# igormq/aes-lac-2018

Measured on AMD Instinct MI355X. Metric: train frames/sec, DeepSpeech2 5xBiGRU-800, higher is better.
Workload: dtype f32

## Files before the change

### aes-lac-2018_amd/csrc/gemm.hip

```cpp
#include <stdlib.h>

#include <type_traits>

#include "ds2_common.h"
#include "split_bf16.h"

namespace {

constexpr int BM = 128, BN = 128, BK = 16;
constexpr int NI = BK / 8;
constexpr int LDT = 132;

constexpr int OOB = 0x7FFFFFF0;
typedef unsigned int u32x4 __attribute__((ext_vector_type(4)));

__device__ __forceinline__ f32x4 bload4(__amdgpu_buffer_rsrc_t rs, int byte_off) {
    return __builtin_bit_cast(f32x4, __builtin_amdgcn_raw_buffer_load_b128(rs, byte_off, 0, 0));
}
__device__ __forceinline__ float bload1(__amdgpu_buffer_rsrc_t rs, int byte_off) {
    return __builtin_bit_cast(float, __builtin_amdgcn_raw_buffer_load_b32(rs, byte_off, 0, 0));
}

template <bool KCONTIG, bool VEC>
__device__ __forceinline__ void load_slab(__amdgpu_buffer_rsrc_t rs, int ld, int x0, int xmax, int k0, int kmax,
                                          int tid, f32x4 (&r)[NI]) {
    if (KCONTIG) {
        const int kq = (tid & (BK / 4 - 1)) * 4;
#pragma unroll
        for (int i = 0; i < NI; ++i) {
            const int x = x0 + tid / (BK / 4) + (1024 / BK) * i;
            const int k = k0 + kq;
            const int off = (x * ld + k) * 4;
            if (VEC) {
                r[i] = bload4(rs, (x < xmax && k + 3 < kmax) ? off : OOB);
            } else {
#pragma unroll
                for (int c = 0; c < 4; ++c) r[i][c] = bload1(rs, (x < xmax && k + c < kmax) ? off + 4 * c : OOB);
            }
        }
    } else {
        const int xq = (tid & 31) * 4;
#pragma unroll
        for (int i = 0; i < NI; ++i) {
            const int k = k0 + (tid >> 5) + 8 * i;
            const int x = x0 + xq;
            const int off = (k * ld + x) * 4;
            if (VEC) {
                if (x + 3 < xmax || x >= xmax) {
                    r[i] = bload4(rs, (k < kmax && x < xmax) ? off : OOB);
                } else {
#pragma unroll
                    for (int c = 0; c < 4; ++c) r[i][c] = bload1(rs, (k < kmax && x + c < xmax) ? off + 4 * c : OOB);
                }
            } else {
#pragma unroll
                for (int c = 0; c < 4; ++c) r[i][c] = bload1(rs, (k < kmax && x + c < xmax) ? off + 4 * c : OOB);
            }
        }
    }
}

template <bool KCONTIG>
__device__ __forceinline__ void slab_voffsets(int ld, int x0, int xmax, int tid, int (&voff)[NI]) {
#pragma unroll
    for (int i = 0; i < NI; ++i) {
        if (KCONTIG) {
            const int x = x0 + tid / (BK / 4) + (1024 / BK) * i;
            voff[i] = x < xmax ? (x * ld + (tid & (BK / 4 - 1)) * 4) * 4 : OOB;
        } else {
            const int x = x0 + (tid & 31) * 4;
            voff[i] = x < xmax ? (((tid >> 5) + 8 * i) * ld + x) * 4 : OOB;
        }
    }
}
template <bool KCONTIG>
__device__ __forceinline__ int slab_soffset(int ld, int k0) {
    return KCONTIG ? k0 * 4 : k0 * ld * 4;
}
__device__ __forceinline__ void load_slab_fast(__amdgpu_buffer_rsrc_t rs, const int (&voff)[NI], int soff, f32x4 (&r)[NI]) {
#pragma unroll
    for (int i = 0; i < NI; ++i)
        r[i] = __builtin_bit_cast(f32x4, __builtin_amdgcn_raw_buffer_load_b128(rs, voff[i], soff, 0));
}

template <bool KCONTIG>
__device__ __forceinline__ void store_slab(float* __restrict__ lds, int tid, const f32x4 (&r)[NI]) {
    if (KCONTIG) {
        const int kq = (tid & (BK / 4 - 1)) * 4;
#pragma unroll
        for (int i = 0; i < NI; ++i) {
            const int x = tid / (BK / 4) + (1024 / BK) * i;
#pragma unroll
            for (int c = 0; c < 4; ++c) lds[(kq + c) * LDT + x] = r[i][c];
        }
    } else {
        const int xq = (tid & 31) * 4;
#pragma unroll
        for (int i = 0; i < NI; ++i) {
            const int k = (tid >> 5) + 8 * i;
            *reinterpret_cast<f32x4*>(&lds[k * LDT + xq]) = r[i];
        }
    }
}

__device__ __forceinline__ int xcd_tile(int wg, int nwg) {
    const int xcd = wg & 7, idx = wg >> 3;
    const int qd = nwg >> 3, rm = nwg & 7;
    return (xcd < rm ? xcd * (qd + 1) : rm * (qd + 1) + (xcd - rm) * qd) + idx;
}

template <bool A_KCONTIG, bool B_KCONTIG, bool VEC, int MODE>
__device__ __forceinline__ void gemm_tile_body(float (&lds)[2][2][BK * LDT], int M, int N, const float* __restrict__ A, int lda,
                                               const float* __restrict__ B, int ldb, float* __restrict__ C, int ldc,
                                               float beta, int use_atomic, unsigned int a_bytes, unsigned int b_bytes, int m0,
                                               int n0, int kbeg, int kend) {
    const int tid = threadIdx.x;
    const int lane = tid & 63;
    const int wave = tid >> 6;
    const int wm = wave >> 1, wn = wave & 1;
    constexpr int NI_ = MODE == 0 ? 2 : 1, NJ_ = MODE == 0 ? 2 : MODE;
    const int arow = MODE == 0 ? wm * 64 : wave * 32, bcol = MODE == 0 ? wn * 64 : 0;

    f32x16 acc[NI_][NJ_];
#pragma unroll
    for (int i = 0; i < NI_; ++i)
#pragma unroll
        for (int j = 0; j < NJ_; ++j)
#pragma unroll
            for (int r = 0; r < 16; ++r) acc[i][j][r] = 0.f;

    const __amdgpu_buffer_rsrc_t rsa = __builtin_amdgcn_make_buffer_rsrc(const_cast<float*>(A), 0, a_bytes, 0x00020000);
    const __amdgpu_buffer_rsrc_t rsb = __builtin_amdgcn_make_buffer_rsrc(const_cast<float*>(B), 0, b_bytes, 0x00020000);
    f32x4 ra[NI], rb[NI];
    const int nslab = (kend - kbeg + BK - 1) / BK;
    if (nslab > 0) {
        load_slab<A_KCONTIG, VEC>(rsa, lda, m0, M, kbeg, kend, tid, ra);
        load_slab<B_KCONTIG, VEC>(rsb, ldb, n0, N, kbeg, kend, tid, rb);
        store_slab<A_KCONTIG>(lds[0][0], tid, ra);
        store_slab<B_KCONTIG>(lds[0][1], tid, rb);
    }
    __syncthreads();

    const int lr = lane & 31, lh = lane >> 5;
    for (int s = 0; s < nslab; ++s) {
        const int cur = s & 1;
#ifndef DS2_GEMM_ABL
#define DS2_GEMM_ABL 0
#endif
        if (s + 1 < nslab && !(DS2_GEMM_ABL & 2)) {
            load_slab<A_KCONTIG, VEC>(rsa, lda, m0, M, kbeg + (s + 1) * BK, kend, tid, ra);
            load_slab<B_KCONTIG, VEC>(rsb, ldb, n0, N, kbeg + (s + 1) * BK, kend, tid, rb);
        }
        const float* as = lds[cur][0] + arow + lr;
        const float* bs = lds[cur][1] + bcol + lr;
#pragma unroll
        for (int kk = 0; kk < BK; kk += 2) {
            float a[NI_], b[NJ_];
#pragma unroll
            for (int i = 0; i < NI_; ++i) a[i] = (DS2_GEMM_ABL & 4) ? ra[0][0] + kk : as[(kk + lh) * LDT + 32 * i];
#pragma unroll
            for (int j = 0; j < NJ_; ++j) b[j] = (DS2_GEMM_ABL & 4) ? rb[0][0] + kk : bs[(kk + lh) * LDT + 32 * j];
#pragma unroll
            for (int i = 0; i < NI_; ++i)
#pragma unroll
                for (int j = 0; j < NJ_; ++j) acc[i][j] = __builtin_amdgcn_mfma_f32_32x32x2f32(a[i], b[j], acc[i][j], 0, 0, 0);
        }
        if (s + 1 < nslab && !(DS2_GEMM_ABL & 1)) {
            store_slab<A_KCONTIG>(lds[cur ^ 1][0], tid, ra);
            store_slab<B_KCONTIG>(lds[cur ^ 1][1], tid, rb);
        }
        __syncthreads();
    }

#pragma unroll
    for (int i = 0; i < NI_; ++i)
#pragma unroll
        for (int j = 0; j < NJ_; ++j) {
            const int n = n0 + bcol + j * 32 + lr;
            if (n >= N) continue;
#pragma unroll
            for (int r = 0; r < 16; ++r) {
                const int m = m0 + arow + i * 32 + (r & 3) + 8 * (r >> 2) + 4 * lh;
                if (m < M) {
                    float* c = C + (size_t)m * ldc + n;
                    if (use_atomic)
                        atomicAdd(c, acc[i][j][r]);
                    else
                        *c = (beta != 0.f) ? acc[i][j][r] + beta * (*c) : acc[i][j][r];
                }
            }
        }
}

template <bool A_KCONTIG, bool B_KCONTIG, bool VEC>
__device__ __forceinline__ void gemm_tile(int M, int N, int K, const float* __restrict__ A, int lda,
                                          const float* __restrict__ B, int ldb, float* __restrict__ C, int ldc, float beta,
                                          int tiles_n, int k_per_split, int use_atomic, unsigned int a_bytes,
                                          unsigned int b_bytes, int tile, int split) {
    __shared__ __attribute__((aligned(16))) float lds[2][2][BK * LDT];
    const int m0 = (tile / tiles_n) * BM;
    const int n0 = (tile % tiles_n) * BN;
    const int kbeg = split * k_per_split;
    const int kend = min(K, kbeg + k_per_split);
    const int ncols = N - n0;
    if (ncols <= 32)
        gemm_tile_body<A_KCONTIG, B_KCONTIG, VEC, 1>(lds, M, N, A, lda, B, ldb, C, ldc, beta, use_atomic, a_bytes, b_bytes, m0,
                                                     n0, kbeg, kend);
    else if (ncols <= 64)
        gemm_tile_body<A_KCONTIG, B_KCONTIG, VEC, 2>(lds, M, N, A, lda, B, ldb, C, ldc, beta, use_atomic, a_bytes, b_bytes, m0,
                                                     n0, kbeg, kend);
    else
        gemm_tile_body<A_KCONTIG, B_KCONTIG, VEC, 0>(lds, M, N, A, lda, B, ldb, C, ldc, beta, use_atomic, a_bytes, b_bytes, m0,
                                                     n0, kbeg, kend);
}

template <bool A_KCONTIG, bool B_KCONTIG, bool VEC>
__global__ __launch_bounds__(256, 2) void gemm_f32_kernel(int M, int N, int K, const float* __restrict__ A,
                                                          int lda, const float* __restrict__ B, int ldb,
                                                          float* __restrict__ C, int ldc, float beta,
                                                          int tiles_n, int k_per_split, int use_atomic,
                                                          unsigned int a_bytes, unsigned int b_bytes) {
    gemm_tile<A_KCONTIG, B_KCONTIG, VEC>(M, N, K, A, lda, B, ldb, C, ldc, beta, tiles_n, k_per_split, use_atomic, a_bytes,
                                         b_bytes, xcd_tile(blockIdx.x, gridDim.x), blockIdx.y);
}

struct GemmGroup {
    const float* A[4];
    const float* B[4];
    float* C[4];
    int M[4], lda[4], ldb[4], ldc[4];
    unsigned int a_bytes[4], b_bytes[4];
};
template <bool VEC>
__global__ __launch_bounds__(256, 2) void gemm_f32_tn_group_kernel(GemmGroup g, int N, int K, int tiles_n, int k_per_split) {
    const int p = blockIdx.z;
    const int tiles = ((g.M[p] + BM - 1) / BM) * tiles_n;
    if ((int)blockIdx.x >= tiles) return;
    gemm_tile<false, false, VEC>(g.M[p], N, K, g.A[p], g.lda[p], g.B[p], g.ldb[p], g.C[p], g.ldc[p], 0.f, tiles_n, k_per_split,
                                 1, g.a_bytes[p], g.b_bytes[p], blockIdx.x, blockIdx.y);
}

template <bool A_KCONTIG, bool B_KCONTIG, bool VEC>
__global__ __launch_bounds__(256, 2) void gemm_f32_v2_kernel(int M, int N, int K, const float* __restrict__ A, int lda,
                                                             const float* __restrict__ B, int ldb,
                                                             float* __restrict__ C, int ldc, float beta, int tiles_n,
                                                             int dp_tiles, int sk_units, int sk_total,
                                                             unsigned int a_bytes, unsigned int b_bytes) {
    __shared__ __attribute__((aligned(16))) float lds[3][2][BK * LDT];
    const int tid = threadIdx.x, lane = tid & 63, wave = tid >> 6;
    const int wm = wave >> 1, wn = wave & 1;
    const int lr = lane & 31, lh = lane >> 5;
    const int nslab_all = (K + BK - 1) / BK;
    const __amdgpu_buffer_rsrc_t rsa = __builtin_amdgcn_make_buffer_rsrc(const_cast<float*>(A), 0, a_bytes, 0x00020000);
    const __amdgpu_buffer_rsrc_t rsb = __builtin_amdgcn_make_buffer_rsrc(const_cast<float*>(B), 0, b_bytes, 0x00020000);

    int u0 = 0, u1 = 0;
    const bool is_dp = (int)blockIdx.x < dp_tiles;
    if (!is_dp) {
        u0 = ((int)blockIdx.x - dp_tiles) * sk_units;
        u1 = min(u0 + sk_units, sk_total);
    }
#pragma unroll 1
    for (int piece = 0; piece < 2; ++piece) {
        int tile, s_beg, s_end;
        if (is_dp) {
            if (piece == 1) break;
            const int nwg = dp_tiles, xcd = blockIdx.x & 7, idx = blockIdx.x >> 3;
            const int qd = nwg >> 3, rm = nwg & 7;
            tile = (xcd < rm ? xcd * (qd + 1) : rm * (qd + 1) + (xcd - rm) * qd) + idx;
            s_beg = 0;
            s_end = nslab_all;
        } else {
            if (u0 >= u1) break;
            tile = dp_tiles + u0 / nslab_all;
            s_beg = u0 % nslab_all;
            s_end = min(nslab_all, s_beg + (u1 - u0));
            u0 += s_end - s_beg;
        }
        const int m0 = (tile / tiles_n) * BM, n0 = (tile % tiles_n) * BN;
        const int nslab = s_end - s_beg;
        const int kbeg = s_beg * BK, kend = min(K, s_end * BK);

        f32x16 acc[2][2];
#pragma unroll
        for (int i = 0; i < 2; ++i)
#pragma unroll
            for (int j = 0; j < 2; ++j)
#pragma unroll
                for (int r = 0; r < 16; ++r) acc[i][j][r] = 0.f;

        f32x4 ra[NI], rb[NI];
        int va[NI], vb[NI];
        slab_voffsets<A_KCONTIG>(lda, m0, M, tid, va);
        slab_voffsets<B_KCONTIG>(ldb, n0, N, tid, vb);
        const bool fast_ok = VEC && (A_KCONTIG || (M & 3) == 0) && (B_KCONTIG || (N & 3) == 0);
        auto fetch = [&](int k0) {
            if (fast_ok && k0 + BK <= kend) {
                load_slab_fast(rsa, va, slab_soffset<A_KCONTIG>(lda, k0), ra);
                load_slab_fast(rsb, vb, slab_soffset<B_KCONTIG>(ldb, k0), rb);
            } else {
                load_slab<A_KCONTIG, VEC>(rsa, lda, m0, M, k0, kend, tid, ra);
                load_slab<B_KCONTIG, VEC>(rsb, ldb, n0, N, k0, kend, tid, rb);
            }
        };
        __syncthreads();
        fetch(kbeg);
        store_slab<A_KCONTIG>(lds[0][0], tid, ra);
        store_slab<B_KCONTIG>(lds[0][1], tid, rb);
        if (nslab > 1) {
            fetch(kbeg + BK);
            store_slab<A_KCONTIG>(lds[1][0], tid, ra);
            store_slab<B_KCONTIG>(lds[1][1], tid, rb);
        }
        if (nslab > 2) {
            fetch(kbeg + 2 * BK);
        }
        __syncthreads();
        const int aoff = wm * 64 + lr + lh * LDT, boff = wn * 64 + lr + lh * LDT;
        float pa0 = lds[0][0][aoff], pa1 = lds[0][0][aoff + 32], pb0 = lds[0][1][boff], pb1 = lds[0][1][boff + 32];
        int cur = 0;
        for (int s = 0; s < nslab; ++s) {
            const float* as = lds[cur][0] + aoff;
            const float* bs = lds[cur][1] + boff;
            const int nxt = cur == 2 ? 0 : cur + 1, nx2 = nxt == 2 ? 0 : nxt + 1;
#pragma unroll
            for (int kk = 0; kk < BK; kk += 2) {
                const float a0 = pa0, a1 = pa1, b0 = pb0, b1 = pb1;
                if (kk + 2 < BK) {
                    pa0 = as[(kk + 2) * LDT];
                    pa1 = as[(kk + 2) * LDT + 32];
                    pb0 = bs[(kk + 2) * LDT];
                    pb1 = bs[(kk + 2) * LDT + 32];
                }
                acc[0][0] = __builtin_amdgcn_mfma_f32_32x32x2f32(a0, b0, acc[0][0], 0, 0, 0);
                acc[0][1] = __builtin_amdgcn_mfma_f32_32x32x2f32(a0, b1, acc[0][1], 0, 0, 0);
                acc[1][0] = __builtin_amdgcn_mfma_f32_32x32x2f32(a1, b0, acc[1][0], 0, 0, 0);
                acc[1][1] = __builtin_amdgcn_mfma_f32_32x32x2f32(a1, b1, acc[1][1], 0, 0, 0);
                __builtin_amdgcn_sched_group_barrier(0x100, 2, 0);
                __builtin_amdgcn_sched_group_barrier(0x008, 4, 0);
                if (kk == BK - 6 && s + 2 < nslab) {
                    store_slab<A_KCONTIG>(lds[nx2][0], tid, ra);
                    store_slab<B_KCONTIG>(lds[nx2][1], tid, rb);
                    if (s + 3 < nslab) fetch(kbeg + (s + 3) * BK);
                }
            }
            if (s + 1 < nslab) {
                pa0 = lds[nxt][0][aoff];
                pa1 = lds[nxt][0][aoff + 32];
                pb0 = lds[nxt][1][boff];
                pb1 = lds[nxt][1][boff + 32];
            }
            __syncthreads();
            cur = nxt;
        }

        const bool atomic = !is_dp;
#pragma unroll
        for (int i = 0; i < 2; ++i)
#pragma unroll
            for (int j = 0; j < 2; ++j) {
                const int n = n0 + wn * 64 + j * 32 + lr;
                if (n >= N) continue;
#pragma unroll
                for (int r = 0; r < 16; ++r) {
                    const int m = m0 + wm * 64 + i * 32 + (r & 3) + 8 * (r >> 2) + 4 * lh;
                    if (m < M) {
                        float* c = C + (size_t)m * ldc + n;
                        if (atomic)
                            atomicAdd(c, acc[i][j][r]);
                        else
                            *c = (beta != 0.f) ? acc[i][j][r] + beta * (*c) : acc[i][j][r];
                    }
                }
            }
    }
}

constexpr int SP = SPLIT_PITCH;
constexpr int SPLIT_TILE_BYTES = 128 * SP;

template <bool KCONTIG>
__device__ __forceinline__ void split_voffsets(int ld, int x0, int xmax, int tid, int (&voff)[2]) {
    if (KCONTIG) {
#pragma unroll
        for (int i = 0; i < 2; ++i) {
            const int x = x0 + (tid >> 2) + 64 * i;
            voff[i] = x < xmax ? (x * ld + (tid & 3) * 4) * 4 : OOB;
        }
    } else {
        const int x = x0 + (tid & 127);
        voff[0] = voff[1] = x < xmax ? (8 * (tid >> 7) * ld + x) * 4 : OOB;
    }
}
template <bool KCONTIG>
__device__ __forceinline__ void split_load(__amdgpu_buffer_rsrc_t rs, const int (&voff)[2], int ld, int k0, float (&r)[8]) {
    if (KCONTIG) {
#pragma unroll
        for (int i = 0; i < 2; ++i) {
            const f32x4 v = __builtin_bit_cast(f32x4, __builtin_amdgcn_raw_buffer_load_b128(rs, voff[i], k0 * 4, 0));
#pragma unroll
            for (int c = 0; c < 4; ++c) r[4 * i + c] = v[c];
        }
    } else {
#pragma unroll
        for (int c = 0; c < 8; ++c)
            r[c] = __builtin_bit_cast(float, __builtin_amdgcn_raw_buffer_load_b32(rs, voff[0], (k0 + c) * ld * 4, 0));
    }
}
template <bool KCONTIG>
__device__ __forceinline__ void split_store(char* __restrict__ lds, int tid, const float (&r)[8]) {
    if (KCONTIG) {
#pragma unroll
        for (int i = 0; i < 2; ++i) {
            unsigned int p[3][2];
            split3(r[4 * i], r[4 * i + 1], p[0][0], p[1][0], p[2][0]);
            split3(r[4 * i + 2], r[4 * i + 3], p[0][1], p[1][1], p[2][1]);
            char* row = lds + ((tid >> 2) + 64 * i) * SP + (tid & 3) * 8;
#pragma unroll
            for (int q = 0; q < 3; ++q) *reinterpret_cast<uint2*>(row + 32 * q) = make_uint2(p[q][0], p[q][1]);
        }
    } else {
        unsigned int p[3][4];
#pragma unroll
        for (int c = 0; c < 4; ++c) split3(r[2 * c], r[2 * c + 1], p[0][c], p[1][c], p[2][c]);
        char* row = lds + (tid & 127) * SP + (tid >> 7) * 16;
#pragma unroll
        for (int q = 0; q < 3; ++q) *reinterpret_cast<uint4*>(row + 32 * q) = make_uint4(p[q][0], p[q][1], p[q][2], p[q][3]);
    }
}

template <bool A_KCONTIG, bool B_KCONTIG, int MODE, int NPROD>
__device__ __forceinline__ void gemm_split_tile_body(char (&lds)[2][2][SPLIT_TILE_BYTES], int M, int N,
                                                     const float* __restrict__ A, int lda, const float* __restrict__ B,
                                                     int ldb, float* __restrict__ C, int ldc, float beta, int use_atomic,
                                                     unsigned int a_bytes, unsigned int b_bytes, int m0, int n0, int kbeg,
                                                     int kend) {
    const int tid = threadIdx.x;
    const int lane = tid & 63;
    const int wave = tid >> 6;
    const int wm = wave >> 1, wn = wave & 1;
    constexpr int NI_ = MODE == 0 ? 2 : 1, NJ_ = MODE == 0 ? 2 : MODE;
    const int arow = MODE == 0 ? wm * 64 : wave * 32, bcol = MODE == 0 ? wn * 64 : 0;

    f32x16 acc[NI_][NJ_], acc_lo[NI_][NJ_];
#pragma unroll
    for (int i = 0; i < NI_; ++i)
#pragma unroll
        for (int j = 0; j < NJ_; ++j)
#pragma unroll
            for (int r = 0; r < 16; ++r) acc[i][j][r] = acc_lo[i][j][r] = 0.f;

    const __amdgpu_buffer_rsrc_t rsa = __builtin_amdgcn_make_buffer_rsrc(const_cast<float*>(A), 0, a_bytes, 0x00020000);
    const __amdgpu_buffer_rsrc_t rsb = __builtin_amdgcn_make_buffer_rsrc(const_cast<float*>(B), 0, b_bytes, 0x00020000);
    float ra[2][8], rb[2][8];
    int va[2], vb[2];
    split_voffsets<A_KCONTIG>(lda, m0, M, tid, va);
    split_voffsets<B_KCONTIG>(ldb, n0, N, tid, vb);
    const int nslab = (kend - kbeg + BK - 1) / BK;
    if (nslab > 0) {
        split_load<A_KCONTIG>(rsa, va, lda, kbeg, ra[0]);
        split_load<B_KCONTIG>(rsb, vb, ldb, kbeg, rb[0]);
    }
    if (nslab > 1) {
        split_load<A_KCONTIG>(rsa, va, lda, kbeg + BK, ra[1]);
        split_load<B_KCONTIG>(rsb, vb, ldb, kbeg + BK, rb[1]);
    }
    if (nslab > 0) {
        split_store<A_KCONTIG>(lds[0][0], tid, ra[0]);
        split_store<B_KCONTIG>(lds[0][1], tid, rb[0]);
    }
    __syncthreads();

    const int lr = lane & 31, lh = lane >> 5;
    const int a_off = (arow + lr) * SP + lh * 16, b_off = (bcol + lr) * SP + lh * 16;
    auto slab = [&](int s, auto PAR) {
        constexpr int cur = decltype(PAR)::value;
        if (!(DS2_GEMM_ABL & 2)) {
        split_load<A_KCONTIG>(rsa, va, lda, kbeg + (s + 2) * BK, ra[cur]);
        split_load<B_KCONTIG>(rsb, vb, ldb, kbeg + (s + 2) * BK, rb[cur]);
        }
        const char* as = lds[cur][0] + a_off;
        const char* bs = lds[cur][1] + b_off;
        bf16x8 a[NI_][3], b[NJ_][3];
#pragma unroll
        for (int i = 0; i < NI_; ++i)
#pragma unroll
            for (int q = 0; q < 3; ++q)
                a[i][q] = (DS2_GEMM_ABL & 4) ? __builtin_bit_cast(bf16x8, f32x4{ra[0][0] + q, ra[0][1], ra[0][2], ra[0][3] + i})
                                             : *reinterpret_cast<const bf16x8*>(as + i * 32 * SP + q * 32);
#pragma unroll
        for (int j = 0; j < NJ_; ++j)
#pragma unroll
            for (int q = 0; q < 3; ++q)
                b[j][q] = (DS2_GEMM_ABL & 4) ? __builtin_bit_cast(bf16x8, f32x4{rb[0][0] + q, rb[0][1], rb[0][2], rb[0][3] + j})
                                             : *reinterpret_cast<const bf16x8*>(bs + j * 32 * SP + q * 32);
#pragma unroll
        for (int i = 0; i < NI_; ++i)
#pragma unroll
            for (int j = 0; j < NJ_; ++j) {
                split_mfma2<NPROD>(a[i], b[j], acc[i][j], acc_lo[i][j]);
            }
        if (!(DS2_GEMM_ABL & 1)) {
        split_store<A_KCONTIG>(lds[cur ^ 1][0], tid, ra[cur ^ 1]);
        split_store<B_KCONTIG>(lds[cur ^ 1][1], tid, rb[cur ^ 1]);
        }
        constexpr int NMFMA = NI_ * NJ_ * NPROD, VPM = (96 + NMFMA - 1) / NMFMA, WEVERY = NMFMA >= 8 ? NMFMA / 8 : 1;
        __builtin_amdgcn_sched_group_barrier(0x020, (A_KCONTIG ? 2 : 8) + (B_KCONTIG ? 2 : 8), 0);
        __builtin_amdgcn_sched_group_barrier(0x100, 3 * (NI_ + NJ_), 0);
#pragma unroll
        for (int g = 0; g < NMFMA; ++g) {
            __builtin_amdgcn_sched_group_barrier(0x008, 1, 0);
            __builtin_amdgcn_sched_group_barrier(0x002, VPM, 0);
            if (g % WEVERY == WEVERY - 1) __builtin_amdgcn_sched_group_barrier(0x200, NMFMA >= 8 ? 1 : 8 / NMFMA + 1, 0);
        }
        __syncthreads();
    };
    for (int s = 0; s < nslab; s += 2) {
        slab(s, std::integral_constant<int, 0>{});
        if (s + 1 < nslab) slab(s + 1, std::integral_constant<int, 1>{});
    }
#pragma unroll
    for (int i = 0; i < NI_; ++i)
#pragma unroll
        for (int j = 0; j < NJ_; ++j)
#pragma unroll
            for (int r = 0; r < 16; ++r) acc[i][j][r] += acc_lo[i][j][r];

#pragma unroll
    for (int i = 0; i < NI_; ++i)
#pragma unroll
        for (int j = 0; j < NJ_; ++j) {
            const int n = n0 + bcol + j * 32 + lr;
            if (n >= N) continue;
#pragma unroll
            for (int r = 0; r < 16; ++r) {
                const int m = m0 + arow + i * 32 + (r & 3) + 8 * (r >> 2) + 4 * lh;
                if (m < M) {
                    float* c = C + (size_t)m * ldc + n;
                    if (use_atomic)
                        atomicAdd(c, acc[i][j][r]);
                    else
                        *c = (beta != 0.f) ? acc[i][j][r] + beta * (*c) : acc[i][j][r];
                }
            }
        }
}

template <bool A_KCONTIG, bool B_KCONTIG, int NPROD>
__device__ __forceinline__ void gemm_split_tile(int M, int N, int K, const float* __restrict__ A, int lda,
                                                const float* __restrict__ B, int ldb, float* __restrict__ C, int ldc,
                                                float beta, int tiles_n, int k_per_split, int use_atomic,
                                                unsigned int a_bytes, unsigned int b_bytes, int tile, int split) {
    __shared__ __attribute__((aligned(16))) char lds[2][2][SPLIT_TILE_BYTES];
    const int m0 = (tile / tiles_n) * BM;
    const int n0 = (tile % tiles_n) * BN;
    const int kbeg = split * k_per_split;
    const int kend = min(K, kbeg + k_per_split);
    const int ncols = N - n0;
    if (ncols <= 32)
        gemm_split_tile_body<A_KCONTIG, B_KCONTIG, 1, NPROD>(lds, M, N, A, lda, B, ldb, C, ldc, beta, use_atomic, a_bytes,
                                                             b_bytes, m0, n0, kbeg, kend);
    else if (ncols <= 64)
        gemm_split_tile_body<A_KCONTIG, B_KCONTIG, 2, NPROD>(lds, M, N, A, lda, B, ldb, C, ldc, beta, use_atomic, a_bytes,
                                                             b_bytes, m0, n0, kbeg, kend);
    else
        gemm_split_tile_body<A_KCONTIG, B_KCONTIG, 0, NPROD>(lds, M, N, A, lda, B, ldb, C, ldc, beta, use_atomic, a_bytes,
                                                             b_bytes, m0, n0, kbeg, kend);
}

template <bool A_KCONTIG, bool B_KCONTIG, int NPROD>
__global__ __launch_bounds__(256, 2) void gemm_bf16x_kernel(int M, int N, int K, const float* __restrict__ A, int lda,
                                                            const float* __restrict__ B, int ldb, float* __restrict__ C,
                                                            int ldc, float beta, int tiles_n, int k_per_split,
                                                            int use_atomic, unsigned int a_bytes, unsigned int b_bytes) {
    gemm_split_tile<A_KCONTIG, B_KCONTIG, NPROD>(M, N, K, A, lda, B, ldb, C, ldc, beta, tiles_n, k_per_split, use_atomic,
                                                 a_bytes, b_bytes, xcd_tile(blockIdx.x, gridDim.x), blockIdx.y);
}
template <int NPROD>
__global__ __launch_bounds__(256, 2) void gemm_bf16x_tn_group_kernel(GemmGroup g, int N, int K, int tiles_n, int k_per_split) {
    const int p = blockIdx.z;
    const int tiles = ((g.M[p] + BM - 1) / BM) * tiles_n;
    if ((int)blockIdx.x >= tiles) return;
    gemm_split_tile<false, false, NPROD>(g.M[p], N, K, g.A[p], g.lda[p], g.B[p], g.ldb[p], g.C[p], g.ldc[p], 0.f, tiles_n,
                                         k_per_split, 1, g.a_bytes[p], g.b_bytes[p], blockIdx.x, blockIdx.y);
}

inline int& gemm_split_mode_ref() {
    static int mode = [] {
        const char* e = getenv("DS2_GEMM_SPLIT");
        const int v = e ? atoi(e) : 6;
        return (v == 6 || v == 9) ? v : 0;
    }();
    return mode;
}
inline int gemm_split_mode() { return gemm_split_mode_ref(); }

inline void zero_rows(float* C, int ldc, int N, int rows, hipStream_t st) {
    if (rows <= 0) return;
    if (ldc == N)
        (void)hipMemsetAsync(C, 0, (size_t)rows * N * sizeof(float), st);
    else
        (void)hipMemset2DAsync(C, (size_t)ldc * sizeof(float), 0, (size_t)N * sizeof(float), rows, st);
}

inline int gemm_slots() {
    static int slots[64] = {0};
    int dev = 0;
    if (hipGetDevice(&dev) != hipSuccess || dev < 0 || dev >= 64) return 512;
    if (slots[dev] == 0) {
        int n = 0;
        if (hipDeviceGetAttribute(&n, hipDeviceAttributeMultiprocessorCount, dev) != hipSuccess || n <= 0) n = 256;
        slots[dev] = 2 * n;
    }
    return slots[dev];
}

template <bool AK, bool BKc>
int launch(int M, int N, int K, const float* A, int lda, const float* B, int ldb, float* C, int ldc, float beta,
           int split_k, hipStream_t st) {
    const int tm = ds2_cdiv(M, BM), tn = ds2_cdiv(N, BN);
    if (split_k == 0) {
        const int tiles = tm * tn;
        split_k = 1;
        if ((tiles < 512 && K >= 512) || (tiles < 2048 && K >= 2048)) {
            static const int env_target = ds2_tune_env("DS2_GEMM_SPLIT_TARGET") ? atoi(ds2_tune_env("DS2_GEMM_SPLIT_TARGET")) : 0;
            const int target = env_target > 0 ? env_target : (gemm_split_mode() != 0 ? 1024 : 8192);
            split_k = target / tiles;
            const int max_split = K / 320 > 1 ? K / 320 : 1;
            if (split_k > max_split) split_k = max_split;
            if (split_k > 32) split_k = 32;
        }
    }
    if (split_k < 1) split_k = 1;
    if (gemm_split_mode() != 0 && (lda % 4 == 0) && (ldb % 4 == 0) && (((uintptr_t)A & 15) == 0) && (((uintptr_t)B & 15) == 0) &&
        ((!AK && !BKc) || K % BK == 0)) {
        int kper = ds2_cdiv(ds2_cdiv(K, split_k), BK) * BK;
        if (kper < BK) kper = BK;
        const int nsplit = ds2_cdiv(K, kper);
        const unsigned long long abytes = 4ull * (AK ? (unsigned long long)(M - 1) * lda + K : (unsigned long long)(K - 1) * lda + M);
        const unsigned long long bbytes = 4ull * (BKc ? (unsigned long long)(N - 1) * ldb + K : (unsigned long long)(K - 1) * ldb + N);
        if (abytes >= 0x7FFFFFF0ull || bbytes >= 0x7FFFFFF0ull) return -1;
        dim3 grid(tm * tn, nsplit), block(256);
        const int atomic = nsplit > 1 ? 1 : 0;
        if (atomic && beta == 0.f) zero_rows(C, ldc, N, M, st);
        if (gemm_split_mode() == 6)
            hipLaunchKernelGGL((gemm_bf16x_kernel<AK, BKc, 6>), grid, block, 0, st, M, N, K, A, lda, B, ldb, C, ldc, beta, tn,
                               kper, atomic, (unsigned int)abytes, (unsigned int)bbytes);
        else
            hipLaunchKernelGGL((gemm_bf16x_kernel<AK, BKc, 9>), grid, block, 0, st, M, N, K, A, lda, B, ldb, C, ldc, beta, tn,
                               kper, atomic, (unsigned int)abytes, (unsigned int)bbytes);
        return 0;
    }
    const bool vec0 = (lda % 4 == 0) && (ldb % 4 == 0) && (((uintptr_t)A & 15) == 0) && (((uintptr_t)B & 15) == 0) &&
                      ((!AK && !BKc) || K % 4 == 0);
    static const bool v2_on = !(ds2_tune_env("DS2_GEMM_V2") && ds2_tune_env("DS2_GEMM_V2")[0] == '0');
    const int tiles_all = tm * tn, slots_all = gemm_slots();
    if (split_k == 1 && v2_on && tiles_all > slots_all && tiles_all % slots_all != 0 && ds2_cdiv(K, BK) >= 16 && beta == 0.f) {
        const unsigned long long abytes = 4ull * (AK ? (unsigned long long)(M - 1) * lda + K : (unsigned long long)(K - 1) * lda + M);
        const unsigned long long bbytes = 4ull * (BKc ? (unsigned long long)(N - 1) * ldb + K : (unsigned long long)(K - 1) * ldb + N);
        if (abytes >= 0x7FFFFFF0ull || bbytes >= 0x7FFFFFF0ull) return -1;
        const int tiles = tm * tn, slots = gemm_slots(), nslab = ds2_cdiv(K, BK);
        int dp = tiles, sk_wgs = 0, sk_units = 0, sk_total = 0;
        const int rem = tiles % slots;
        const bool hybrid = tiles > slots && rem != 0 && nslab >= 16 && beta == 0.f;
        if (hybrid) {
            dp = tiles - rem;
            sk_total = rem * nslab;
            sk_wgs = sk_total / 16 < slots ? sk_total / 16 : slots;
            if (sk_wgs < 1) sk_wgs = 1;
            sk_units = ds2_cdiv(sk_total, sk_wgs);
            if (sk_units > nslab) {
                sk_units = nslab;
            }
            sk_wgs = ds2_cdiv(sk_total, sk_units);
            const int r0 = (dp / tn) * BM;
            zero_rows(C + (size_t)r0 * ldc, ldc, N, M - r0, st);
        }
        dim3 grid(dp + sk_wgs), block(256);
        if (vec0)
            hipLaunchKernelGGL((gemm_f32_v2_kernel<AK, BKc, true>), grid, block, 0, st, M, N, K, A, lda, B, ldb, C, ldc,
                               beta, tn, dp, sk_units, sk_total, (unsigned int)abytes, (unsigned int)bbytes);
        else
            hipLaunchKernelGGL((gemm_f32_v2_kernel<AK, BKc, false>), grid, block, 0, st, M, N, K, A, lda, B, ldb, C, ldc,
                               beta, tn, dp, sk_units, sk_total, (unsigned int)abytes, (unsigned int)bbytes);
        return 0;
    }
    int kper = ds2_cdiv(ds2_cdiv(K, split_k), BK) * BK;
    if (kper < BK) kper = BK;
    const int nsplit = ds2_cdiv(K, kper);
    const bool vec = (lda % 4 == 0) && (ldb % 4 == 0) && (((uintptr_t)A & 15) == 0) && (((uintptr_t)B & 15) == 0) &&
                     ((!AK && !BKc) || K % 4 == 0);
    const unsigned long long abytes = 4ull * (AK ? (unsigned long long)(M - 1) * lda + K : (unsigned long long)(K - 1) * lda + M);
    const unsigned long long bbytes = 4ull * (BKc ? (unsigned long long)(N - 1) * ldb + K : (unsigned long long)(K - 1) * ldb + N);
    if (abytes >= 0x7FFFFFF0ull || bbytes >= 0x7FFFFFF0ull) return -1;
    dim3 grid(tm * tn, nsplit), block(256);
    const int atomic = nsplit > 1 ? 1 : 0;
    if (atomic && beta == 0.f)
        zero_rows(C, ldc, N, M, st);
    if (vec)
        hipLaunchKernelGGL((gemm_f32_kernel<AK, BKc, true>), grid, block, 0, st, M, N, K, A, lda, B, ldb, C, ldc,
                           beta, tn, kper, atomic, (unsigned int)abytes, (unsigned int)bbytes);
    else
        hipLaunchKernelGGL((gemm_f32_kernel<AK, BKc, false>), grid, block, 0, st, M, N, K, A, lda, B, ldb, C, ldc,
                           beta, tn, kper, atomic, (unsigned int)abytes, (unsigned int)bbytes);
    return 0;
}

}

extern "C" int ds2_gemm_f32(int trans_a, int trans_b, int M, int N, int K, const float* A, int lda,
                            const float* B, int ldb, float* C, int ldc, float beta, int split_k, void* stream) {
    DS2_CHECK_ARG(M > 0 && N > 0 && K > 0);
    DS2_CHECK_ARG(A && B && C);
    DS2_CHECK_ARG(beta == 0.f || beta == 1.f);
    DS2_CHECK_ARG(split_k >= 0);
    DS2_CHECK_ARG(lda >= (trans_a ? M : K) && ldb >= (trans_b ? K : N) && ldc >= N);
    hipStream_t st = (hipStream_t)stream;
    int rc;
    if (!trans_a && !trans_b) rc = launch<true, false>(M, N, K, A, lda, B, ldb, C, ldc, beta, split_k, st);
    else if (!trans_a && trans_b) rc = launch<true, true>(M, N, K, A, lda, B, ldb, C, ldc, beta, split_k, st);
    else if (trans_a && !trans_b) rc = launch<false, false>(M, N, K, A, lda, B, ldb, C, ldc, beta, split_k, st);
    else rc = launch<false, true>(M, N, K, A, lda, B, ldb, C, ldc, beta, split_k, st);
    if (rc != 0) {
        ds2_set_error("ds2_gemm_f32: operand larger than 2 GB is not supported");
        return DS2_ERR_UNSUPPORTED;
    }
    DS2_CHECK_LAUNCH();
    return DS2_OK;
}

extern "C" int ds2_gemm_split_mode(int mode) {
    if (mode == 0 || mode == 6 || mode == 9) gemm_split_mode_ref() = mode;
    return gemm_split_mode();
}

extern "C" int ds2_gemm_f32_tn_group(int count, const float* const* A_host, const int* lda_host, const int* M_host,
                                     const float* const* B_host, const int* ldb_host, float* const* C_host,
                                     const int* ldc_host, int N, int K, int accumulate, void* stream) {
    DS2_CHECK_ARG(count >= 1 && count <= 4 && A_host && lda_host && M_host && B_host && ldb_host && C_host && ldc_host);
    DS2_CHECK_ARG(N > 0 && K > 0);
    GemmGroup g;
    int max_tiles = 0, tot_tiles = 0;
    const int tn = ds2_cdiv(N, BN);
    bool vec = true;
    for (int p = 0; p < 4; ++p) {
        const int q = p < count ? p : 0;
        DS2_CHECK_ARG(A_host[q] && B_host[q] && C_host[q] && M_host[q] > 0 && lda_host[q] >= M_host[q] && ldb_host[q] >= N &&
                      ldc_host[q] >= N);
        g.A[p] = A_host[q];
        g.B[p] = B_host[q];
        g.C[p] = C_host[q];
        g.M[p] = M_host[q];
        g.lda[p] = lda_host[q];
        g.ldb[p] = ldb_host[q];
        g.ldc[p] = ldc_host[q];
        const unsigned long long ab = 4ull * ((unsigned long long)(K - 1) * lda_host[q] + M_host[q]);
        const unsigned long long bb = 4ull * ((unsigned long long)(K - 1) * ldb_host[q] + N);
        if (ab >= 0x7FFFFFF0ull || bb >= 0x7FFFFFF0ull) {
            ds2_set_error("ds2_gemm_f32_tn_group: operand larger than 2 GB is not supported");
            return DS2_ERR_UNSUPPORTED;
        }
        g.a_bytes[p] = (unsigned int)ab;
        g.b_bytes[p] = (unsigned int)bb;
        vec = vec && (lda_host[q] % 4 == 0) && (ldb_host[q] % 4 == 0) && (((uintptr_t)A_host[q] & 15) == 0) &&
              (((uintptr_t)B_host[q] & 15) == 0);
        if (p < count) {
            const int t = ds2_cdiv(M_host[q], BM) * tn;
            tot_tiles += t;
            if (t > max_tiles) max_tiles = t;
        }
    }
    int split_k = 1;
    if (tot_tiles < 512 && K >= 512) {
        static const int env_target = ds2_tune_env("DS2_GEMM_GROUP_TARGET") ? atoi(ds2_tune_env("DS2_GEMM_GROUP_TARGET")) : 0;
        const int target = env_target > 0 ? env_target : (gemm_split_mode() != 0 ? 1024 : 3072);
        split_k = target / tot_tiles;
        const int max_split = K / 320 > 1 ? K / 320 : 1;
        if (split_k > max_split) split_k = max_split;
        if (split_k > 32) split_k = 32;
        if (split_k < 1) split_k = 1;
    }
    int kper = ds2_cdiv(ds2_cdiv(K, split_k), BK) * BK;
    if (kper < BK) kper = BK;
    const int nsplit = ds2_cdiv(K, kper);
    hipStream_t st = (hipStream_t)stream;
    for (int p = 0; p < count && !accumulate; ++p)
        zero_rows(g.C[p], g.ldc[p], N, g.M[p], st);
    dim3 grid(max_tiles, nsplit, count), block(256);
    if (vec && gemm_split_mode() == 6)
        hipLaunchKernelGGL((gemm_bf16x_tn_group_kernel<6>), grid, block, 0, st, g, N, K, tn, kper);
    else if (vec && gemm_split_mode() == 9)
        hipLaunchKernelGGL((gemm_bf16x_tn_group_kernel<9>), grid, block, 0, st, g, N, K, tn, kper);
    else if (vec)
        hipLaunchKernelGGL((gemm_f32_tn_group_kernel<true>), grid, block, 0, st, g, N, K, tn, kper);
    else
        hipLaunchKernelGGL((gemm_f32_tn_group_kernel<false>), grid, block, 0, st, g, N, K, tn, kper);
    DS2_CHECK_LAUNCH();
    return DS2_OK;
}
```

Baseline: 545,800.

## Vectorize x-contiguous GEMM operand loads with k-major LDS image and transpose reads

Adds a third operand form for the split-bf16 GEMM when the operand is contiguous along M/N instead of K. Each thread now issues two 128-bit buffer loads instead of eight scalar loads, stores the split bf16 planes into a k-major, XOR-swizzled LDS image, and uses ds_read_tr16_b64 transpose reads to build the MFMA fragments. The aim is to cut global load instruction count and improve coalescing for transposed operands, at the cost of twice as many LDS read instructions per fragment and padded buffer bounds. The path is on by default and can be turned off with an environment variable.

```diff
diff --git a/aes-lac-2018_amd/csrc/gemm.hip b/aes-lac-2018_amd/csrc/gemm.hip
--- a/aes-lac-2018_amd/csrc/gemm.hip
+++ b/aes-lac-2018_amd/csrc/gemm.hip
@@ -379,37 +379,50 @@
 constexpr int SP = SPLIT_PITCH;
 constexpr int SPLIT_TILE_BYTES = 128 * SP;
 
-template <bool KCONTIG>
+constexpr int XT_ROW = 256, XT_PLANE = 16 * XT_ROW;
+static_assert(3 * XT_PLANE <= SPLIT_TILE_BYTES, "the k-major image must fit the slab");
+
+template <int FORM>
 __device__ __forceinline__ void split_voffsets(int ld, int x0, int xmax, int tid, int (&voff)[2]) {
-    if (KCONTIG) {
+    if (FORM == 0) {
 #pragma unroll
         for (int i = 0; i < 2; ++i) {
             const int x = x0 + (tid >> 2) + 64 * i;
             voff[i] = x < xmax ? (x * ld + (tid & 3) * 4) * 4 : OOB;
         }
-    } else {
+    } else if (FORM == 1) {
         const int x = x0 + (tid & 127);
         voff[0] = voff[1] = x < xmax ? (8 * (tid >> 7) * ld + x) * 4 : OOB;
-    }
-}
-template <bool KCONTIG>
+    } else {
+        const int x = x0 + 4 * (tid & 31);
+        voff[0] = voff[1] = x < xmax ? ((tid >> 5) * ld + x) * 4 : OOB;
+    }
+}
+template <int FORM>
 __device__ __forceinline__ void split_load(__amdgpu_buffer_rsrc_t rs, const int (&voff)[2], int ld, int k0, float (&r)[8]) {
-    if (KCONTIG) {
+    if (FORM == 0) {
 #pragma unroll
         for (int i = 0; i < 2; ++i) {
             const f32x4 v = __builtin_bit_cast(f32x4, __builtin_amdgcn_raw_buffer_load_b128(rs, voff[i], k0 * 4, 0));
 #pragma unroll
             for (int c = 0; c < 4; ++c) r[4 * i + c] = v[c];
         }
-    } else {
+    } else if (FORM == 1) {
 #pragma unroll
         for (int c = 0; c < 8; ++c)
             r[c] = __builtin_bit_cast(float, __builtin_amdgcn_raw_buffer_load_b32(rs, voff[0], (k0 + c) * ld * 4, 0));
-    }
-}
-template <bool KCONTIG>
+    } else {
+#pragma unroll
+        for (int i = 0; i < 2; ++i) {
+            const f32x4 v = __builtin_bit_cast(f32x4, __builtin_amdgcn_raw_buffer_load_b128(rs, voff[0], (k0 + 8 * i) * ld * 4, 0));
+#pragma unroll
+            for (int c = 0; c < 4; ++c) r[4 * i + c] = v[c];
+        }
+    }
+}
+template <int FORM>
 __device__ __forceinline__ void split_store(char* __restrict__ lds, int tid, const float (&r)[8]) {
-    if (KCONTIG) {
+    if (FORM == 0) {
 #pragma unroll
         for (int i = 0; i < 2; ++i) {
             unsigned int p[3][2];
@@ -419,17 +432,46 @@
 #pragma unroll
             for (int q = 0; q < 3; ++q) *reinterpret_cast<uint2*>(row + 32 * q) = make_uint2(p[q][0], p[q][1]);
         }
-    } else {
+    } else if (FORM == 1) {
         unsigned int p[3][4];
 #pragma unroll
         for (int c = 0; c < 4; ++c) split3(r[2 * c], r[2 * c + 1], p[0][c], p[1][c], p[2][c]);
         char* row = lds + (tid & 127) * SP + (tid >> 7) * 16;
 #pragma unroll
         for (int q = 0; q < 3; ++q) *reinterpret_cast<uint4*>(row + 32 * q) = make_uint4(p[q][0], p[q][1], p[q][2], p[q][3]);
-    }
-}
-
-template <bool A_KCONTIG, bool B_KCONTIG, int MODE, int NPROD>
+    } else {
+        const int k = tid >> 5;
+        char* row = lds + k * XT_ROW + ((8 * (tid & 31)) ^ ((k & 3) << 6));
+#pragma unroll
+        for (int i = 0; i < 2; ++i) {
+            unsigned int p[3][2];
+            split3(r[4 * i], r[4 * i + 1], p[0][0], p[1][0], p[2][0]);
+            split3(r[4 * i + 2], r[4 * i + 3], p[0][1], p[1][1], p[2][1]);
+#pragma unroll
+            for (int q = 0; q < 3; ++q)
+                *reinterpret_cast<uint2*>(row + 8 * i * XT_ROW + q * XT_PLANE) = make_uint2(p[q][0], p[q][1]);
+        }
+    }
+}
+template <int FORM>
+__device__ __forceinline__ int split_frag_offset(int xbase, int lane) {
+    const int lr = lane & 31, lh = lane >> 5;
+    if (FORM != 2) return (xbase + lr) * SP + lh * 16;
+    const int q = (lane >> 2) & 3, p = lane & 3, g = (lane >> 4) & 1;
+    return (8 * lh + q) * XT_ROW + ((2 * xbase) ^ (q << 6)) + 32 * g + 8 * p;
+}
+template <int FORM>
+__device__ __forceinline__ bf16x8 split_frag_read(const char* p, int plane) {
+    if (FORM != 2) return *reinterpret_cast<const bf16x8*>(p + plane * 32);
+    typedef short s16x4 __attribute__((ext_vector_type(4)));
+    typedef __attribute__((address_space(3))) s16x4* lds_s16x4_ptr;
+    const s16x4 lo = __builtin_amdgcn_ds_read_tr16_b64_v4i16((lds_s16x4_ptr)(p + plane * XT_PLANE));
+    const s16x4 hi = __builtin_amdgcn_ds_read_tr16_b64_v4i16((lds_s16x4_ptr)(p + plane * XT_PLANE + 4 * XT_ROW));
+    typedef short s16x8 __attribute__((ext_vector_type(8)));
+    return __builtin_bit_cast(bf16x8, (s16x8)__builtin_shufflevector(lo, hi, 0, 1, 2, 3, 4, 5, 6, 7));
+}
+
+template <int FA, int FB, int MODE, int NPROD>
 __device__ __forceinline__ void gemm_split_tile_body(char (&lds)[2][2][SPLIT_TILE_BYTES], int M, int N,
                                                      const float* __restrict__ A, int lda, const float* __restrict__ B,
                                                      int ldb, float* __restrict__ C, int ldc, float beta, int use_atomic,
@@ -454,46 +496,50 @@
     const __amdgpu_buffer_rsrc_t rsb = __builtin_amdgcn_make_buffer_rsrc(const_cast<float*>(B), 0, b_bytes, 0x00020000);
     float ra[2][8], rb[2][8];
     int va[2], vb[2];
-    split_voffsets<A_KCONTIG>(lda, m0, M, tid, va);
-    split_voffsets<B_KCONTIG>(ldb, n0, N, tid, vb);
+    split_voffsets<FA>(lda, m0, M, tid, va);
+    split_voffsets<FB>(ldb, n0, N, tid, vb);
     const int nslab = (kend - kbeg + BK - 1) / BK;
     if (nslab > 0) {
-        split_load<A_KCONTIG>(rsa, va, lda, kbeg, ra[0]);
-        split_load<B_KCONTIG>(rsb, vb, ldb, kbeg, rb[0]);
+        split_load<FA>(rsa, va, lda, kbeg, ra[0]);
+        split_load<FB>(rsb, vb, ldb, kbeg, rb[0]);
     }
     if (nslab > 1) {
-        split_load<A_KCONTIG>(rsa, va, lda, kbeg + BK, ra[1]);
-        split_load<B_KCONTIG>(rsb, vb, ldb, kbeg + BK, rb[1]);
+        split_load<FA>(rsa, va, lda, kbeg + BK, ra[1]);
+        split_load<FB>(rsb, vb, ldb, kbeg + BK, rb[1]);
     }
     if (nslab > 0) {
-        split_store<A_KCONTIG>(lds[0][0], tid, ra[0]);
-        split_store<B_KCONTIG>(lds[0][1], tid, rb[0]);
+        split_store<FA>(lds[0][0], tid, ra[0]);
+        split_store<FB>(lds[0][1], tid, rb[0]);
     }
     __syncthreads();
 
     const int lr = lane & 31, lh = lane >> 5;
-    const int a_off = (arow + lr) * SP + lh * 16, b_off = (bcol + lr) * SP + lh * 16;
+    int a_off[NI_], b_off[NJ_];
+#pragma unroll
+    for (int i = 0; i < NI_; ++i) a_off[i] = split_frag_offset<FA>(arow + 32 * i, lane);
+#pragma unroll
+    for (int j = 0; j < NJ_; ++j) b_off[j] = split_frag_offset<FB>(bcol + 32 * j, lane);
     auto slab = [&](int s, auto PAR) {
         constexpr int cur = decltype(PAR)::value;
         if (!(DS2_GEMM_ABL & 2)) {
-        split_load<A_KCONTIG>(rsa, va, lda, kbeg + (s + 2) * BK, ra[cur]);
-        split_load<B_KCONTIG>(rsb, vb, ldb, kbeg + (s + 2) * BK, rb[cur]);
-        }
-        const char* as = lds[cur][0] + a_off;
-        const char* bs = lds[cur][1] + b_off;
+        split_load<FA>(rsa, va, lda, kbeg + (s + 2) * BK, ra[cur]);
+        split_load<FB>(rsb, vb, ldb, kbeg + (s + 2) * BK, rb[cur]);
+        }
+        const char* as = lds[cur][0];
+        const char* bs = lds[cur][1];
         bf16x8 a[NI_][3], b[NJ_][3];
 #pragma unroll
         for (int i = 0; i < NI_; ++i)
 #pragma unroll
             for (int q = 0; q < 3; ++q)
                 a[i][q] = (DS2_GEMM_ABL & 4) ? __builtin_bit_cast(bf16x8, f32x4{ra[0][0] + q, ra[0][1], ra[0][2], ra[0][3] + i})
-                                             : *reinterpret_cast<const bf16x8*>(as + i * 32 * SP + q * 32);
+                                             : split_frag_read<FA>(as + a_off[i], q);
 #pragma unroll
         for (int j = 0; j < NJ_; ++j)
 #pragma unroll
             for (int q = 0; q < 3; ++q)
                 b[j][q] = (DS2_GEMM_ABL & 4) ? __builtin_bit_cast(bf16x8, f32x4{rb[0][0] + q, rb[0][1], rb[0][2], rb[0][3] + j})
-                                             : *reinterpret_cast<const bf16x8*>(bs + j * 32 * SP + q * 32);
+                                             : split_frag_read<FB>(bs + b_off[j], q);
 #pragma unroll
         for (int i = 0; i < NI_; ++i)
 #pragma unroll
@@ -501,12 +547,12 @@
                 split_mfma2<NPROD>(a[i], b[j], acc[i][j], acc_lo[i][j]);
             }
         if (!(DS2_GEMM_ABL & 1)) {
-        split_store<A_KCONTIG>(lds[cur ^ 1][0], tid, ra[cur ^ 1]);
-        split_store<B_KCONTIG>(lds[cur ^ 1][1], tid, rb[cur ^ 1]);
+        split_store<FA>(lds[cur ^ 1][0], tid, ra[cur ^ 1]);
+        split_store<FB>(lds[cur ^ 1][1], tid, rb[cur ^ 1]);
         }
         constexpr int NMFMA = NI_ * NJ_ * NPROD, VPM = (96 + NMFMA - 1) / NMFMA, WEVERY = NMFMA >= 8 ? NMFMA / 8 : 1;
-        __builtin_amdgcn_sched_group_barrier(0x020, (A_KCONTIG ? 2 : 8) + (B_KCONTIG ? 2 : 8), 0);
-        __builtin_amdgcn_sched_group_barrier(0x100, 3 * (NI_ + NJ_), 0);
+        __builtin_amdgcn_sched_group_barrier(0x020, (FA == 1 ? 8 : 2) + (FB == 1 ? 8 : 2), 0);
+        __builtin_amdgcn_sched_group_barrier(0x100, (FA == 2 ? 6 : 3) * NI_ + (FB == 2 ? 6 : 3) * NJ_, 0);
 #pragma unroll
         for (int g = 0; g < NMFMA; ++g) {
             __builtin_amdgcn_sched_group_barrier(0x008, 1, 0);
@@ -546,7 +592,7 @@
         }
 }
 
-template <bool A_KCONTIG, bool B_KCONTIG, int NPROD>
+template <int FA, int FB, int NPROD>
 __device__ __forceinline__ void gemm_split_tile(int M, int N, int K, const float* __restrict__ A, int lda,
                                                 const float* __restrict__ B, int ldb, float* __restrict__ C, int ldc,
                                                 float beta, int tiles_n, int k_per_split, int use_atomic,
@@ -558,30 +604,32 @@
     const int kend = min(K, kbeg + k_per_split);
     const int ncols = N - n0;
     if (ncols <= 32)
-        gemm_split_tile_body<A_KCONTIG, B_KCONTIG, 1, NPROD>(lds, M, N, A, lda, B, ldb, C, ldc, beta, use_atomic, a_bytes,
+        gemm_split_tile_body<FA, FB, 1, NPROD>(lds, M, N, A, lda, B, ldb, C, ldc, beta, use_atomic, a_bytes,
                                                              b_bytes, m0, n0, kbeg, kend);
     else if (ncols <= 64)
-        gemm_split_tile_body<A_KCONTIG, B_KCONTIG, 2, NPROD>(lds, M, N, A, lda, B, ldb, C, ldc, beta, use_atomic, a_bytes,
+        gemm_split_tile_body<FA, FB, 2, NPROD>(lds, M, N, A, lda, B, ldb, C, ldc, beta, use_atomic, a_bytes,
                                                              b_bytes, m0, n0, kbeg, kend);
     else
-        gemm_split_tile_body<A_KCONTIG, B_KCONTIG, 0, NPROD>(lds, M, N, A, lda, B, ldb, C, ldc, beta, use_atomic, a_bytes,
+        gemm_split_tile_body<FA, FB, 0, NPROD>(lds, M, N, A, lda, B, ldb, C, ldc, beta, use_atomic, a_bytes,
                                                              b_bytes, m0, n0, kbeg, kend);
 }
 
-template <bool A_KCONTIG, bool B_KCONTIG, int NPROD>
+template <bool A_KCONTIG, bool B_KCONTIG, int NPROD, bool XLOAD>
 __global__ __launch_bounds__(256, 2) void gemm_bf16x_kernel(int M, int N, int K, const float* __restrict__ A, int lda,
                                                             const float* __restrict__ B, int ldb, float* __restrict__ C,
                                                             int ldc, float beta, int tiles_n, int k_per_split,
                                                             int use_atomic, unsigned int a_bytes, unsigned int b_bytes) {
-    gemm_split_tile<A_KCONTIG, B_KCONTIG, NPROD>(M, N, K, A, lda, B, ldb, C, ldc, beta, tiles_n, k_per_split, use_atomic,
-                                                 a_bytes, b_bytes, xcd_tile(blockIdx.x, gridDim.x), blockIdx.y);
-}
-template <int NPROD>
+    constexpr int XF = XLOAD ? 2 : 1;
+    gemm_split_tile<A_KCONTIG ? 0 : XF, B_KCONTIG ? 0 : XF, NPROD>(M, N, K, A, lda, B, ldb, C, ldc, beta, tiles_n, k_per_split,
+                                                                   use_atomic, a_bytes, b_bytes, xcd_tile(blockIdx.x, gridDim.x),
+                                                                   blockIdx.y);
+}
+template <int NPROD, bool XLOAD>
 __global__ __launch_bounds__(256, 2) void gemm_bf16x_tn_group_kernel(GemmGroup g, int N, int K, int tiles_n, int k_per_split) {
     const int p = blockIdx.z;
     const int tiles = ((g.M[p] + BM - 1) / BM) * tiles_n;
     if ((int)blockIdx.x >= tiles) return;
-    gemm_split_tile<false, false, NPROD>(g.M[p], N, K, g.A[p], g.lda[p], g.B[p], g.ldb[p], g.C[p], g.ldc[p], 0.f, tiles_n,
+    gemm_split_tile<XLOAD ? 2 : 1, XLOAD ? 2 : 1, NPROD>(g.M[p], N, K, g.A[p], g.lda[p], g.B[p], g.ldb[p], g.C[p], g.ldc[p], 0.f, tiles_n,
                                          k_per_split, 1, g.a_bytes[p], g.b_bytes[p], blockIdx.x, blockIdx.y);
 }
 
@@ -594,6 +642,16 @@
     return mode;
 }
 inline int gemm_split_mode() { return gemm_split_mode_ref(); }
+inline bool gemm_xload() {
+    static const bool on = [] {
+        const char* e = getenv("DS2_GEMM_XLOAD");
+        return !(e && e[0] == '0');
+    }();
+    return on;
+}
+inline unsigned long long xcontig_bytes(int k, int ld, int width, bool xload) {
+    return 4ull * ((unsigned long long)(k - 1) * ld + (xload ? (width + 3) / 4 * 4 : width));
+}
 
 inline void zero_rows(float* C, int ldc, int N, int rows, hipStream_t st) {
     if (rows <= 0) return;
@@ -637,18 +695,26 @@
         int kper = ds2_cdiv(ds2_cdiv(K, split_k), BK) * BK;
         if (kper < BK) kper = BK;
         const int nsplit = ds2_cdiv(K, kper);
-        const unsigned long long abytes = 4ull * (AK ? (unsigned long long)(M - 1) * lda + K : (unsigned long long)(K - 1) * lda + M);
-        const unsigned long long bbytes = 4ull * (BKc ? (unsigned long long)(N - 1) * ldb + K : (unsigned long long)(K - 1) * ldb + N);
+        const bool xl = gemm_xload();
+        const unsigned long long abytes = AK ? 4ull * ((unsigned long long)(M - 1) * lda + K) : xcontig_bytes(K, lda, M, xl);
+        const unsigned long long bbytes = BKc ? 4ull * ((unsigned long long)(N - 1) * ldb + K) : xcontig_bytes(K, ldb, N, xl);
         if (abytes >= 0x7FFFFFF0ull || bbytes >= 0x7FFFFFF0ull) return -1;
         dim3 grid(tm * tn, nsplit), block(256);
         const int atomic = nsplit > 1 ? 1 : 0;
         if (atomic && beta == 0.f) zero_rows(C, ldc, N, M, st);
-        if (gemm_split_mode() == 6)
-            hipLaunchKernelGGL((gemm_bf16x_kernel<AK, BKc, 6>), grid, block, 0, st, M, N, K, A, lda, B, ldb, C, ldc, beta, tn,
+        constexpr bool XC = !AK || !BKc;
+        if (gemm_split_mode() == 6 && XC && xl)
+            hipLaunchKernelGGL((gemm_bf16x_kernel<AK, BKc, 6, XC>), grid, block, 0, st, M, N, K, A, lda, B, ldb, C, ldc, beta, tn,
+                               kper, atomic, (unsigned int)abytes, (unsigned int)bbytes);
+        else if (gemm_split_mode() == 6)
+            hipLaunchKernelGGL((gemm_bf16x_kernel<AK, BKc, 6, false>), grid, block, 0, st, M, N, K, A, lda, B, ldb, C, ldc, beta,
+                               tn, kper, atomic, (unsigned int)abytes, (unsigned int)bbytes);
+        else if (XC && xl)
+            hipLaunchKernelGGL((gemm_bf16x_kernel<AK, BKc, 9, XC>), grid, block, 0, st, M, N, K, A, lda, B, ldb, C, ldc, beta, tn,
                                kper, atomic, (unsigned int)abytes, (unsigned int)bbytes);
         else
-            hipLaunchKernelGGL((gemm_bf16x_kernel<AK, BKc, 9>), grid, block, 0, st, M, N, K, A, lda, B, ldb, C, ldc, beta, tn,
-                               kper, atomic, (unsigned int)abytes, (unsigned int)bbytes);
+            hipLaunchKernelGGL((gemm_bf16x_kernel<AK, BKc, 9, false>), grid, block, 0, st, M, N, K, A, lda, B, ldb, C, ldc, beta,
+                               tn, kper, atomic, (unsigned int)abytes, (unsigned int)bbytes);
         return 0;
     }
     const bool vec0 = (lda % 4 == 0) && (ldb % 4 == 0) && (((uintptr_t)A & 15) == 0) && (((uintptr_t)B & 15) == 0) &&
@@ -743,6 +809,7 @@
     int max_tiles = 0, tot_tiles = 0;
     const int tn = ds2_cdiv(N, BN);
     bool vec = true;
+    const bool xl = gemm_xload() && gemm_split_mode() != 0;
     for (int p = 0; p < 4; ++p) {
         const int q = p < count ? p : 0;
         DS2_CHECK_ARG(A_host[q] && B_host[q] && C_host[q] && M_host[q] > 0 && lda_host[q] >= M_host[q] && ldb_host[q] >= N &&
@@ -754,16 +821,21 @@
         g.lda[p] = lda_host[q];
         g.ldb[p] = ldb_host[q];
         g.ldc[p] = ldc_host[q];
-        const unsigned long long ab = 4ull * ((unsigned long long)(K - 1) * lda_host[q] + M_host[q]);
-        const unsigned long long bb = 4ull * ((unsigned long long)(K - 1) * ldb_host[q] + N);
+        unsigned long long ab = 4ull * ((unsigned long long)(K - 1) * lda_host[q] + M_host[q]);
+        unsigned long long bb = 4ull * ((unsigned long long)(K - 1) * ldb_host[q] + N);
+        const bool vec_q = (lda_host[q] % 4 == 0) && (ldb_host[q] % 4 == 0) && (((uintptr_t)A_host[q] & 15) == 0) &&
+                           (((uintptr_t)B_host[q] & 15) == 0);
+        if (vec_q && xl) {
+            ab = xcontig_bytes(K, lda_host[q], M_host[q], true);
+            bb = xcontig_bytes(K, ldb_host[q], N, true);
+        }
         if (ab >= 0x7FFFFFF0ull || bb >= 0x7FFFFFF0ull) {
             ds2_set_error("ds2_gemm_f32_tn_group: operand larger than 2 GB is not supported");
             return DS2_ERR_UNSUPPORTED;
         }
         g.a_bytes[p] = (unsigned int)ab;
         g.b_bytes[p] = (unsigned int)bb;
-        vec = vec && (lda_host[q] % 4 == 0) && (ldb_host[q] % 4 == 0) && (((uintptr_t)A_host[q] & 15) == 0) &&
-              (((uintptr_t)B_host[q] & 15) == 0);
+        vec = vec && vec_q;
         if (p < count) {
             const int t = ds2_cdiv(M_host[q], BM) * tn;
             tot_tiles += t;
@@ -787,10 +859,14 @@
     for (int p = 0; p < count && !accumulate; ++p)
         zero_rows(g.C[p], g.ldc[p], N, g.M[p], st);
     dim3 grid(max_tiles, nsplit, count), block(256);
-    if (vec && gemm_split_mode() == 6)
-        hipLaunchKernelGGL((gemm_bf16x_tn_group_kernel<6>), grid, block, 0, st, g, N, K, tn, kper);
+    if (vec && gemm_split_mode() == 6 && xl)
+        hipLaunchKernelGGL((gemm_bf16x_tn_group_kernel<6, true>), grid, block, 0, st, g, N, K, tn, kper);
+    else if (vec && gemm_split_mode() == 6)
+        hipLaunchKernelGGL((gemm_bf16x_tn_group_kernel<6, false>), grid, block, 0, st, g, N, K, tn, kper);
+    else if (vec && gemm_split_mode() == 9 && xl)
+        hipLaunchKernelGGL((gemm_bf16x_tn_group_kernel<9, true>), grid, block, 0, st, g, N, K, tn, kper);
     else if (vec && gemm_split_mode() == 9)
-        hipLaunchKernelGGL((gemm_bf16x_tn_group_kernel<9>), grid, block, 0, st, g, N, K, tn, kper);
+        hipLaunchKernelGGL((gemm_bf16x_tn_group_kernel<9, false>), grid, block, 0, st, g, N, K, tn, kper);
     else if (vec)
         hipLaunchKernelGGL((gemm_f32_tn_group_kernel<true>), grid, block, 0, st, g, N, K, tn, kper);
     else
```

Measured after the change: 544,000. About the same (-0.3%).
